# fanzyflani/pwnfps

Hardware: AMD Instinct MI355X
Metric: Mpixels/s at 3840x2160 (level.txt scene, trace + blur), frames resident on the device; mean steps/ray alongside; d2h_inclusive = the rate with every frame delivered to the host (SURVEY 8d) (higher is better)
Workload: dtype f32; 1 GPU; pwnfps level.txt scene (14 game.lua spheres, spawn pose, sec_current=0), 3840x2160, POSTPROC_BLUR=1, one frame per step; level=pwnfps_level, width=3840, height=2160, blur_passes=1, parallelism=rows/1, 3 frames in flight on two compute streams, frames_repeated_with_whole_strips=0

## Files before the change

### pwnfps_amd/csrc/pwn_api.cpp

```cpp
#include <hip/hip_runtime.h>
#include <stdint.h>
#include <stdio.h>
#include <stdlib.h>
#include <string.h>
#include <time.h>
#include <new>
#include <algorithm>
#include <vector>
#include <xmmintrin.h>

#include "pwnhip.h"
#include "pwn_internal.h"
#include "level_host.h"
#include "approx_tables.inc"

extern "C" const char *pwn_strerror(int code)
{
	switch(code)
	{
		case PWN_OK: return "ok";
		case PWN_EINVAL: return "invalid argument";
		case PWN_ENODEV: return "no usable HIP device";
		case PWN_ENOMEM: return "out of memory";
		case PWN_EIO: return "level file could not be read";
// ... 2 lines not shown
		case PWN_ETOOBIG: return "sphere tables exceed PWN_TABLES_MAX";
		case PWN_EBUSY: return "frame slot still in flight";
		case PWN_ENOTSUP: return "not available (RCCL missing, or not configured)";
		case PWN_ETIMEDOUT: return "the row tiling's deadline passed waiting for a peer";
	}
	return "unknown error";
}

extern "C" const char *pwn_last_error(pwn_ctx *ctx) { return ctx ? ctx->err : "null context"; }

static int ensure_scratch(pwn_ctx *c, size_t bytes)
{
	if(bytes <= c->scratch_cap) return PWN_OK;
	if(c->d_scratch) { (void)hipFree(c->d_scratch); c->d_scratch = NULL; c->scratch_cap = 0; }
	HIPCHK(c, hipMalloc((void **)&c->d_scratch, bytes));
	c->scratch_cap = bytes;
	return PWN_OK;
}

static void expand_tables(uint16_t *rcp, uint16_t *rsq);
static void frames_release(pwn_ctx *c);

#define GRP_HEAD(c) ((c) != NULL && (c)->grp != NULL && (c)->grp_head)
#define GRP_M0(c) pwn_group_member((c), 0)
#define GRP_REFUSE(c, what) do { if(GRP_HEAD(c)) { snprintf((c)->err, sizeof((c)->err), "%s is not available on a group's handle", what); return PWN_ENOTSUP; } } while(0)

extern "C" int pwn_init(pwn_ctx **out, int device, int width, int height)
{
	if(out == NULL || width <= 0 || height <= 0 || width > 32768 || height > 32768) return PWN_EINVAL;
	*out = NULL;
	int ndev = 0;
	if(hipGetDeviceCount(&ndev) != hipSuccess || ndev <= 0 || device < 0 || device >= ndev) return PWN_ENODEV;
	pwn_ctx *c = new(std::nothrow) pwn_ctx();
	if(c == NULL) return PWN_ENOMEM;
	c->device = device; c->w = width; c->h = height;
	c->blur_passes = 1; c->counters_on = 0; c->scheduler = PWN_SCHED_DEFAULT; c->refill_limit = PWN_REFILL_LIMIT_DEFAULT; c->have_level = false; c->cell_base_ok = false;
	if(const char *e = getenv("PWN_SCHEDULER")) c->scheduler = (strcmp(e, "refill") == 0 || strcmp(e, "1") == 0) ? PWN_SCHED_REFILL : PWN_SCHED_UNITS;
	if(const char *e = getenv("PWN_REFILL_LIMIT")) { int v = atoi(e); if(v >= 1 && v <= 64000) c->refill_limit = v; }
	c->dbg_force_hasw = getenv("PWN_DBG_FORCE_HASW") != NULL;
	c->dbg_blocks_per_cu = 0;
	c->dbg_blur_th = 0;
	if(const char *e = getenv("PWN_DBG_BLUR_TH")) c->dbg_blur_th = atoi(e);
	c->dbg_sphere_lists = 0; c->off_recsph = 0;
	c->dbg_sphere_lists = pwn_i_forced_lists();
	c->nbounds = 0;
	{ const char *e = getenv("PWN_SPHERE_BOUNDS"); c->dbg_sphere_bounds = (e != NULL && strcmp(e, "0") == 0) ? 0 : 1; }
	c->lists_form = PWN_LF_INDEXED; c->big_which = c->big_sph = 0; c->big_high = 0;
	for(int i = 0; i < PWN_NBLOB; i++) { c->d_big[i] = NULL; c->d_big_cap[i] = 0; }
	for(int i = 0; i < PWN_NSTAGE; i++) { c->h_big[i] = NULL; c->h_big_cap[i] = 0; }
	c->dbg_blur_tw = 0; c->dbg_blur_batch = -1;
	if(const char *e = getenv("PWN_DBG_BLUR_TW")) c->dbg_blur_tw = atoi(e);
	if(const char *e = getenv("PWN_DBG_BLUR_BATCH")) if(*e) c->dbg_blur_batch = atoi(e);
	if(const char *e = getenv("PWN_DBG_BLOCKS_PER_CU")) { int v = atoi(e); if(v > 0) c->dbg_blocks_per_cu = v; }
	c->blob_cur = 0; c->blob_dirty = true; c->off_sph = 0; c->stage_next = 0; c->up_stream = NULL;
	for(int i = 0; i < PWN_NBLOB; i++)
	{
		c->d_blob[i] = NULL; c->blob_has_static[i] = false;
		c->ev_tables[i] = NULL; c->tables_in_use[i] = false; c->tables_wait[i] = NULL;
		c->ev_upload[i] = NULL; c->upload_pending[i] = false;
	}
	for(int i = 0; i < PWN_NSTAGE; i++) { c->h_stage[i] = NULL; c->ev_stage[i] = NULL; c->stage_used[i] = false; }
	c->d_pre = c->d_out = NULL; c->d_z = NULL; c->d_skip = NULL; c->d_counters = NULL; c->d_tickets = NULL; c->ticket_set = 0; c->launch_rot = 2; c->launch_waits = 0;
	c->grid_reserve = 0;
	c->d_vpre = c->d_vout = NULL; c->d_vz = NULL; c->views_cap = 0; c->h_vrec = c->d_vrec = NULL; c->d_vrec_dev = NULL;
	c->d_ppre = c->d_pout = NULL; c->d_pz = NULL; c->h_prec = c->d_prec = NULL;
	c->h_rays = c->d_rays = NULL; c->rays_cap = 0;
	c->h_hits = c->d_hits = NULL; c->hits_cap = 0;
	memset(&c->room, 0, sizeof(c->room)); c->room.mode = -1;
	if(const char *e = getenv("PWN_TRACE_ROOM")) if(*e) c->room.mode = atoi(e) < 0 ? -1 : atoi(e);
	c->d_scratch = NULL; c->scratch_cap = 0;
	for(int i = 0; i < 12; i++) { c->occ_lds[i] = 0; c->occ_blocks[i] = 0; }
	c->stream = NULL; c->copy_stream = NULL; c->copy_stream2 = NULL; c->stream2 = NULL; c->d_pre2 = NULL;
	c->frame_overlap = 1; c->last_frame_done = NULL; c->last_frame_stream = NULL;
	if(const char *e = getenv("PWN_FRAME_OVERLAP")) c->frame_overlap = atoi(e) != 0;
	c->unit_order = 0;
	if(const char *e = getenv("PWN_UNIT_ORDER")) c->unit_order = atoi(e) != 0;
	c->tiled_comms = PWN_TILED_COMMS_ONE;
	if(const char *e = getenv("PWN_TILED_COMMS")) c->tiled_comms = (strcmp(e, "perstream") == 0 || strcmp(e, "2") == 0) ? PWN_TILED_COMMS_PER_STREAM : PWN_TILED_COMMS_ONE;
	c->tiled_streams = PWN_TILED_STREAMS_DEFAULT;
	if(const char *e = getenv("PWN_TILED_STREAMS")) { const int v = atoi(e); if(v == 2 || v == 3) c->tiled_streams = v; }
	c->tiled_choreo = PWN_TILED_CHOREO_INSTREAM;
	if(const char *e = getenv("PWN_TILED_CHOREO")) c->tiled_choreo = (strcmp(e, "split") == 0 || strcmp(e, "1") == 0) ? PWN_TILED_CHOREO_SPLIT : PWN_TILED_CHOREO_INSTREAM;
	memset(c->ev, 0, sizeof(c->ev));
	memset(&c->stats, 0, sizeof(c->stats));
	c->strip_reach = 0;
	c->call_strips = -1; c->strip_ev_n = 0; c->d_strip_miss = NULL; c->h_strip_miss = NULL; c->strip_backoff = 0;
	c->strip_calls = c->strip_redone = 0; c->strips_last = 1; c->host_regs_n = 0;
	memset(c->strip_ev, 0, sizeof(c->strip_ev));
	c->strip_copy_streams = 0; c->strip_calib_n = 0;
	if(const char *e = getenv("PWN_CALL_COPY_STREAMS")) if(atoi(e) == 1 || atoi(e) == 2) c->strip_copy_streams = atoi(e);
	if(const char *e = getenv("PWN_CALL_STRIPS")) if(*e) { const int v = atoi(e); if(v >= -1 && v <= PWN_CALL_STRIPS_MAX && v != 1) c->call_strips = v; }
	c->frame_timing = 1; c->wave_log_on = 0; c->d_wave_log = NULL; c->wave_log_cap = 0;
	c->nslots = 0; c->frame_flags = 0; c->frame_scale = 1; c->frame_pitch = 0; c->frame_seq = 0;
	memset(c->slot, 0, sizeof(c->slot));
	c->tiled = NULL; c->grp = NULL; c->grp_head = false; c->hub = NULL;
	c->err[0] = 0;
	pwn_level_clear(c->cells, c->pmap, c->spawn);
	c->bin_off.assign(4097, 0);
	expand_tables(c->tabs, c->tabs + 2048);

	int rc = PWN_OK;
	do
	{
		hipDeviceProp_t prop;
		if(hipSetDevice(device) != hipSuccess || hipGetDeviceProperties(&prop, device) != hipSuccess) { rc = PWN_ENODEV; break; }
		if(strncmp(prop.gcnArchName, "gfx950", 6) != 0)
// ... 838 lines not shown
		P.g_sph = (const float *)(c->d_big[cur] + c->big_sph);
	}
	P.nbounds = c->dbg_sphere_bounds ? c->nbounds : 0;
	for(int i = 0; i < PWN_BOUNDS_MAX; i++)
	{
		P.bound_ids[i] = 0xffffffffu;
		if(i < P.nbounds) { P.bounds[i] = c->bounds[i]; P.bound_ids[i] = c->bounds[i].id; }
	}
	if(c->upload_pending[cur])
	{
		if(hipEventQuery(c->ev_upload[cur]) == hipSuccess) c->upload_pending[cur] = false;
		else HIPCHK(c, hipStreamWaitEvent(stream, c->ev_upload[cur], 0));
	}
	P.counters = c->d_counters;
	P.clear_word = L->clear_word;
	P.cost_word = L->cost_word;
	P.wave_log = NULL;
	const unsigned rot = (unsigned)c->launch_rot, nsets = 2u * rot;
	P.tickets = c->d_tickets + (c->ticket_set % nsets) * PWN_QUEUES * PWN_QUEUE_STRIDE;
	P.tickets_next = c->d_tickets + ((c->ticket_set + rot) % nsets) * PWN_QUEUES * PWN_QUEUE_STRIDE;
	if(views != NULL) P.has_w = views->has_w;
	else if(rays != NULL) P.has_w = rays->has_w;
	else if(vps != NULL) P.has_w = vps->has_w;
	else P.has_w = camera_has_w(L->cam);
	if(c->dbg_force_hasw) P.has_w = 1;
	if(c->counters_on) HIPCHK(c, hipMemsetAsync(c->d_counters, 0, PWN_NCOUNTERS * sizeof(unsigned long long), stream));
	const bool refill = c->scheduler == PWN_SCHED_REFILL && !batch && !glb;
	const size_t lds_bytes = ((P.blob_bytes + 15u) & ~15u) + (refill ? pwn_trace_refill_lds_extra(P.has_w != 0) : pwn_trace_lds_extra());
	P.scheduler = c->scheduler;
	P.refill_limit = c->refill_limit;
	const int variant = (glb ? 8 : 0) | (refill ? 4 : 0) | (c->counters_on ? 2 : 0) | (P.has_w ? 1 : 0);
	if(c->occ_lds[variant] != lds_bytes)
	{
		c->occ_blocks[variant] = refill ? pwn_trace_refill_blocks_per_cu(lds_bytes, c->counters_on != 0, P.has_w != 0)
		                       : glb ? pwn_trace_global_blocks_per_cu(lds_bytes, c->counters_on != 0, P.has_w != 0)
		                             : pwn_trace_blocks_per_cu(lds_bytes, c->counters_on != 0, P.has_w != 0);
		c->occ_lds[variant] = lds_bytes;
	}
	int per_cu = c->occ_blocks[variant];
	{
		const int lds_fit = (int)(155648u / (((uint32_t)lds_bytes + 2047u) & ~2047u));
		if(per_cu > lds_fit) per_cu = lds_fit;
	}
	if(per_cu < 1) per_cu = 1;
	if(c->dbg_blocks_per_cu > 0) per_cu = c->dbg_blocks_per_cu;
	int grid = c->num_cus * per_cu;
	{
		const int room = c->room.mode >= 0 ? c->room.mode : L->room;
		const int reserve = c->grid_reserve > room ? c->grid_reserve : room;
		L->cost_mul = (uint32_t)grid;
		if(reserve > 0 && grid > 2 * reserve) grid -= reserve;
		L->cost_div = (uint32_t)grid;
	}
	{
		const int wg_waves = 4;
		if(!refill && grid > (P.tiles_total + wg_waves - 1) / wg_waves) grid = (P.tiles_total + wg_waves - 1) / wg_waves;
		if(grid > P.tiles_total) grid = P.tiles_total;
	}
	if(c->wave_log_on && !batch)
	{
		const size_t entries = (size_t)grid * 4 + 1;
		if(entries > c->wave_log_cap)
		{
			if(c->d_wave_log) { HIPCHK(c, hipDeviceSynchronize()); (void)hipFree(c->d_wave_log); c->d_wave_log = NULL; c->wave_log_cap = 0; }
			HIPCHK(c, hipMalloc((void **)&c->d_wave_log, entries * 16));
			c->wave_log_cap = entries;
		}
		HIPCHK(c, hipMemsetAsync(c->d_wave_log, 0, c->wave_log_cap * 16, stream));
		P.wave_log = c->d_wave_log;
	}
	const bool want_cost = !refill && !batch && !glb && (c->unit_order || (c->wave_log_on && getenv("PWN_DBG_UNIT_COST") != NULL));
	pwn_ctx::unit_order_state *uop = batch ? NULL : order_entry(c, stream, want_cost);
	if(uop != NULL && want_cost)
	{
		pwn_ctx::unit_order_state &uo = *uop;
		const size_t units = (size_t)P.tiles_total;
		const uint32_t qcap = (uint32_t)((units + PWN_QUEUES - 1u) / PWN_QUEUES);
		if(units > uo.cost_cap || (size_t)qcap * PWN_QUEUES > uo.perm_cap)
		{
			if(uo.d_cost || uo.d_perm) HIPCHK(c, hipDeviceSynchronize());
			(void)hipFree(uo.d_cost); (void)hipFree(uo.d_perm);
			uo.d_cost = NULL; uo.d_perm = NULL; uo.cost_cap = uo.perm_cap = 0; uo.perm_valid = uo.cost_fresh = false;
			HIPCHK(c, hipMalloc((void **)&uo.d_cost, units * 2));
			HIPCHK(c, hipMalloc((void **)&uo.d_perm, (size_t)qcap * PWN_QUEUES * 4));
			uo.cost_cap = units; uo.perm_cap = (size_t)qcap * PWN_QUEUES;
		}
		P.unit_cost = uo.d_cost;
		if(c->unit_order && uo.perm_valid && uo.perm_units == (uint32_t)units && uo.perm_y0 == y0 && uo.perm_y1 == y1)
		{
			P.perm = uo.d_perm; P.perm_cap = qcap;
			c->order_used++;
		}
		uo.units = (uint32_t)units; uo.qcap = qcap; uo.y0 = y0; uo.y1 = y1; uo.cost_fresh = true;
	}
	else if(uop != NULL) uop->cost_fresh = false;
	if(c->launch_event[rot - 1] != NULL && c->launch_stream[rot - 1] != stream)
	{
		HIPCHK(c, hipStreamWaitEvent(stream, c->launch_event[rot - 1], 0));
		c->launch_waits++;
	}
	if(refill) HIPCHK(c, pwn_launch_trace_refill(&P, grid, lds_bytes, c->counters_on != 0, stream));
	else HIPCHK(c, pwn_launch_trace(&P, grid, lds_bytes, c->counters_on != 0, stream));
	c->ticket_set++;
	c->launch_stream[2] = c->launch_stream[1]; c->launch_event[2] = c->launch_event[1];
	c->launch_stream[1] = c->launch_stream[0]; c->launch_event[1] = c->launch_event[0];
	c->launch_stream[0] = stream; c->launch_event[0] = caller_event != NULL ? caller_event : c->ev_tables[cur];
	if(caller_event != NULL)
	{
		for(int i = 0; i < PWN_NBLOB; i++)
			if(c->tables_in_use[i] && c->tables_wait[i] == caller_event) c->tables_in_use[i] = false;
		c->tables_wait[cur] = caller_event;
	}
	else
	{
		HIPCHK(c, hipEventRecord(c->ev_tables[cur], stream));
		c->tables_wait[cur] = c->ev_tables[cur];
	}
	c->tables_in_use[cur] = true;
	return PWN_OK;
}

int pwn_i_launch_order(pwn_ctx *c, hipStream_t stream)
{
	pwn_ctx::unit_order_state *uop = order_entry(c, stream, false);
// ... 1032 lines not shown
```

### pwnfps_amd/csrc/pwn_internal.h

```cpp
#pragma once
#include <hip/hip_runtime.h>
#include <stdint.h>
#include <stdio.h>
#include <vector>
#include <atomic>

#include "pwnhip.h"
#include "tables.h"

struct pwn_views_launch
{
	const pwn_view_rec *d_recs;
	int n;
	bool has_w;
	unsigned long long plane;
};

struct pwn_vps_launch
{
	const pwn_viewport_rec *d_recs, *h_recs;
	int n;
	bool has_w;
	uint32_t units;
};
// ... 124 lines not shown

	uint8_t cells[4096];
	uint32_t cell_base[65 * 65];
	bool cell_base_ok;
	uint32_t ep_recs[PWN_EP_MAX];
	pwn_portal pmap[26];
	int32_t spawn[2];
	std::vector<pwn_sphere> spheres;
	std::vector<int32_t> bin_off, bin_idx;
	std::vector<pwn_sphere> objs;
	std::vector<uint8_t> obj_typ;

	std::vector<uint8_t> blob;
	uint8_t *d_blob[PWN_NBLOB]; int blob_cur;
	bool blob_has_static[PWN_NBLOB];
	hipEvent_t ev_tables[PWN_NBLOB]; bool tables_in_use[PWN_NBLOB];
	hipEvent_t tables_wait[PWN_NBLOB];
	hipEvent_t ev_upload[PWN_NBLOB]; bool upload_pending[PWN_NBLOB];
	uint8_t *h_stage[PWN_NSTAGE]; hipEvent_t ev_stage[PWN_NSTAGE]; bool stage_used[PWN_NSTAGE]; unsigned stage_next;
	hipStream_t up_stream;
	uint16_t tabs[4096];
	uint32_t off_sph;
	uint32_t off_recsph; int dbg_sphere_lists;
	int lists_form;
	pwn_sphere_bound bounds[PWN_BOUNDS_MAX]; int nbounds;
	int dbg_sphere_bounds;
	std::vector<uint8_t> big; uint64_t big_which, big_sph;
	uint8_t *d_big[PWN_NBLOB]; size_t d_big_cap[PWN_NBLOB];
	uint8_t *h_big[PWN_NSTAGE]; size_t h_big_cap[PWN_NSTAGE];
	size_t big_high;
	bool blob_dirty;
	size_t occ_lds[12]; int occ_blocks[12];

	uint32_t *d_pre, *d_out;
	float *d_z;
	uint2 *d_skip;
	unsigned long long *d_counters;
	unsigned long long *d_wave_log; int wave_log_on; size_t wave_log_cap;
	struct unit_order_state
	{
		hipStream_t key; bool used; unsigned long long stamp;
		uint16_t *d_cost; uint32_t *d_perm; size_t cost_cap, perm_cap;
		uint32_t units, qcap; int y0, y1;
		bool cost_fresh;
		uint32_t perm_units; int perm_y0, perm_y1; bool perm_valid;
	} order[4];
	unsigned long long order_stamp;
	int tiled_choreo;
	int tiled_streams;
	int tiled_comms;
	int unit_order;
	unsigned long long order_used, order_sorts;
	bool dbg_force_hasw; int dbg_blocks_per_cu;
	int dbg_blur_th, dbg_blur_tw, dbg_blur_batch;
	int grid_reserve;
	uint32_t *d_vpre, *d_vout; float *d_vz; int views_cap;
	pwn_view_rec *h_vrec, *d_vrec;
	pwn_view_rec *d_vrec_dev;
	uint32_t *d_ppre, *d_pout; float *d_pz;
	pwn_viewport_rec *h_prec, *d_prec;
	unsigned char *h_rays, *d_rays; size_t rays_cap;
	unsigned char *h_hits, *d_hits; size_t hits_cap;
	uint32_t *d_tickets; unsigned ticket_set;
	uint32_t *d_scratch; size_t scratch_cap;

	hipStream_t stream;
	hipStream_t stream2;
	uint32_t *d_pre2;
	pwn_room_ctl room;
	int frame_overlap;
	hipEvent_t last_frame_done; hipStream_t last_frame_stream;
	hipStream_t copy_stream;
	hipEvent_t ev[4];
	int call_strips;
	hipStream_t copy_stream2;
	int strip_copy_streams;
	int strip_calib_n; double strip_calib_ms[16];
	hipEvent_t strip_ev[2 * PWN_CALL_STRIPS_MAX]; int strip_ev_n;
	uint32_t *d_strip_miss, *h_strip_miss;
	int strips_last;
	int strip_reach;
	int strip_backoff;
	unsigned long long strip_calls, strip_redone;
	struct host_reg { void *base; size_t bytes; } host_regs[PWN_HOST_REGS_MAX]; int host_regs_n;
	pwn_stats stats;

	int nslots, frame_flags, frame_scale, frame_pitch, frame_timing;
	pwn_slot slot[PWN_MAX_SLOTS];
	uint64_t frame_seq;

	pwn_group *grp; bool grp_head;
	pwn_hub *hub;
	pwn_tiled *tiled;
	int tiled_init_ms, tiled_wait_ms;

	hipStream_t launch_stream[3]; hipEvent_t launch_event[3];
	unsigned long long launch_waits;
	int launch_rot;

	char err[256];
};

#define HIPCHK(ctx, call) do { hipError_t e_ = (call); if(e_ != hipSuccess) { \
	snprintf((ctx)->err, sizeof((ctx)->err), "%s: %s", #call, hipGetErrorString(e_)); return PWN_EHIP; } } while(0)

int pwn_i_launch_trace(pwn_ctx *c, pwn_trace_launch *L);
// ... 44 lines not shown
```

### pwnfps_amd/csrc/tables.h

```cpp
#pragma once
#include <stdint.h>
#include "cell_bake.h"
#include "sphere_bound.h"

#define PWN_GRID_PITCH 65u
#define PWN_T_RCP      0u
#define PWN_T_RSQ      4096u
#define PWN_T_FACES    8192u
#define PWN_T_EXP2     8448u
#define PWN_T_CELLINFO 8704u
#define PWN_T_EPREC    25616u
#define PWN_T_BINIDX   25824u

#define PWN_RCP_BASE   0x7e800000u
#define PWN_RSQ_BASE   0x5f000000u

#define PWN_C_ROOM   0x0100u
#define PWN_C_ROOM2  0x0200u
#define PWN_C_FOG    0x0400u
#define PWN_C_DQ     0x0800u
#define PWN_C_RAMP   0x1000u
#define PWN_C_RAMPX  0x2000u
#define PWN_C_RAMPM  0x4000u
#define PWN_C_PORTAL 0x8000u
// ... 57 lines not shown
		case '$': return PWN_C_ROOM | PWN_C_FOG;
		case '"': return PWN_C_ROOM | PWN_C_DQ;
		case '#': return PWN_C_ROOM | PWN_C_ROOM2;
		case '&': return PWN_C_ROOM | PWN_C_ROOM2 | PWN_C_FOG;
		case '>': return PWN_C_RAMP | PWN_C_RAMPX | PWN_C_RAMPM;
		case '<': return PWN_C_RAMP | PWN_C_RAMPX;
		case ',': return PWN_C_RAMP | PWN_C_RAMPM;
		case '^': return PWN_C_RAMP;
	}
	return (c >= 'A' && c <= 'Z') ? PWN_C_PORTAL : 0u;
}

struct pwn_trace_params
{
	float rayb[4], rdx[4], rdy[4], from[4];
	float sec_current;
	int w, h, y0, y1;
	int tiles_x, tiles_total;
	uint32_t ux_magic; int ux_shift;
	uint32_t blob_bytes, off_sph;
	uint32_t *sbuf;
	float *zbuf;
	const uint32_t *blob;
	unsigned long long *counters;
	unsigned long long *wave_log;
	int has_w;
	int scheduler;
	int refill_limit;
	uint32_t *tickets, *tickets_next;
	uint32_t *cost_word;
	uint16_t *unit_cost;
	const uint32_t *perm;
	uint32_t perm_cap;
	uint32_t *clear_word;
	uint32_t off_recsph;
	const struct pwn_view_rec *views;
	int nviews;
	uint32_t views_magic; int views_shift;
	unsigned long long plane;
	const float *rays;
	const uint32_t *ray_seeds;
	uint32_t nrays;
	int ray_w;
	void *hits;
	const float *g_rec;
	const uint32_t *g_which;
	const float *g_sph;
	const struct pwn_viewport_rec *vps;
	int nvp;
	uint32_t vp_step0;
	int nbounds;
	uint32_t bound_ids[PWN_BOUNDS_MAX];
	pwn_sphere_bound bounds[PWN_BOUNDS_MAX];
};
#define PWN_HIT_REC_BYTES 48u

struct pwn_blur_params
{
	int w, h, y0, y1;
	int groups;
	const uint32_t *pre;
	const float *zbuf;
	uint32_t *out;
	const uint2 *skip;
	int avail_y0, avail_y1;
	uint32_t *miss;
	int tile_h, tile_w, batch;
	uint32_t *cost_acc, *cost_out;
	uint32_t cost_mul, cost_div;
	int views;
	unsigned long long plane;
	const struct pwn_viewport_rec *vps;
	int nvp, vp_tiles;
};

enum { PWN_KM_FRAME = 0, PWN_KM_VIEWS = 1, PWN_KM_RAYS = 2, PWN_KM_HITS = 3, PWN_KM_VIEWPORTS = 4 };

struct pwn_view_rec
{
	float rayb[4], rdx[4], rdy[4], from[4];
	float sec_current;
	float pad_[3];
};
#define PWN_VIEWS_REC_BYTES 80u

struct pwn_viewport_rec
{
	float rayb[4], rdx[4], rdy[4], from[4];
	float sec_current;
	int32_t x, y, w, h;
	uint32_t units_x; uint32_t ux_magic; int32_t ux_shift;
	uint32_t rows_u;
	uint32_t units;
	uint32_t seg_first, seg_round, seg_magic; int32_t seg_shift;
	uint32_t pad_[2];
};
#define PWN_VP_REC_BYTES 128u

#ifndef PWN_QUEUES
#define PWN_QUEUES 64u
#endif
#define PWN_QUEUE_STRIDE 32u
```

### pwnfps_amd/csrc/trace_common.h

```cpp
#pragma once
#include <hip/hip_runtime.h>
#include <mutex>
#include "dev_math.h"
#include "tables.h"

#define EPS 0.0000000000001f
#define REFLECT_BLUR_F 0.03f
#define REFLECT_MAX 2
enum { FXP = 0, FZP, FXN, FZN, FYP, FYN };

#ifndef PWN_BLOCK
#define PWN_BLOCK 256
#endif
#define TILE_W 16
#define TILE_H 4

#ifndef PWN_MIN_WAVES
#define PWN_MIN_WAVES 3
#endif

#define PWN_LDS __attribute__((address_space(3)))
#define PWN_KARGS __attribute__((address_space(4)))
template<class T> __device__ __forceinline__ const PWN_LDS T *lds_at(uint32_t byte) { return (const PWN_LDS T *)(uintptr_t)byte; }
typedef float pwn_f4 __attribute__((ext_vector_type(4)));
// ... 62 lines not shown

static_assert(PWN_C_PST_SHIFT == 2u && PWN_T_EPREC + PWN_EP_MAX * 4u <= PWN_T_BINIDX, "ep_rec takes the state field as a byte offset; 52 records fit");
static_assert(PWN_C_RAMPX == (1u << PWN_C_PROT_SHIFT) && PWN_C_RAMPM == (2u << PWN_C_PROT_SHIFT), "the rotation takes the place of RAMPX | RAMPM");
static_assert(pwn_cell_class('A') == PWN_C_PORTAL && pwn_cell_class('M') == PWN_C_PORTAL && pwn_cell_class('Z') == PWN_C_PORTAL, "a letter's cell has no ramp bit");
static_assert((PWN_C_PST_MASK | PWN_C_LT2 | PWN_C_LTDQ) == 0xffu, "the baked byte lies below the class bits");
typedef _Float16 pwn_h2 __attribute__((ext_vector_type(2)));
__device__ __forceinline__ pwn_h2 ep_rec(const Lds &L, uint32_t pst_in_place)
{
	return __builtin_bit_cast(pwn_h2, *(const PWN_LDS uint32_t *)(L.eprec + pst_in_place));
}

template<bool HAS_W> struct Vec { float x, y, z, w; };

template<bool W> __device__ __forceinline__ float dot3(const Vec<W> &a, const Vec<W> &b)
{
	if constexpr(W) return (a.x * b.x + a.z * b.z) + (a.y * b.y + a.w * b.w);
	else return (a.x * b.x + a.z * b.z) + a.y * b.y;
}
template<bool W> __device__ __forceinline__ Vec<W> vscale(float s, const Vec<W> &a)
{
	Vec<W> r; r.x = s * a.x; r.y = s * a.y; r.z = s * a.z;
	if constexpr(W) r.w = s * a.w; else r.w = 0.0f;
	return r;
}
template<bool W> __device__ __forceinline__ Vec<W> vadd(const Vec<W> &a, const Vec<W> &b)
{
	Vec<W> r; r.x = a.x + b.x; r.y = a.y + b.y; r.z = a.z + b.z;
	if constexpr(W) r.w = a.w + b.w; else r.w = 0.0f;
	return r;
}
template<bool W> __device__ __forceinline__ Vec<W> vsub(const Vec<W> &a, const Vec<W> &b)
{
	Vec<W> r; r.x = a.x - b.x; r.y = a.y - b.y; r.z = a.z - b.z;
	if constexpr(W) r.w = a.w - b.w; else r.w = 0.0f;
	return r;
}
template<bool W> __device__ __forceinline__ Vec<W> vnormalise(const PWN_LDS uint16_t *rsq, const Vec<W> &a)
{
	return vscale<W>(tab_rsqrt(rsq, dot3<W>(a, a)), a);
}

__device__ __forceinline__ float dpp_row_shr1(float v)
{
	return __int_as_float(__builtin_amdgcn_update_dpp(0, __float_as_int(v), 0x111 , 0xf, 0xf, true));
}

enum { EV_NONE = 0, EV_WALL, EV_SPHERE, EV_EXHAUSTED };
enum { BASE_CEIL = 0, BASE_FLOOR, BASE_WALL, BASE_MAGENTA, BASE_ROOM_Y };

enum { RG_SEG = 0, RG_SETUP_SLOW, RG_EXHAUSTED, RG_WALL, RG_SPHERE, RG_FLOOR, RG_SPHREFL, RG_JITTER, RG_COMP1, RG_COMP1_FOG,
	RG_COMP2, RG_COMP2_FOG, RG_HELP, RG_UNIT, RG_SPHTEST, RG_SPHUPD, RG_ELSE,
	RG_UNIT_HALF, RG_HC_R2, RG_HC_OUT, RG_PORTAL_WALL, RG_PORTAL_GO, RG_PORTAL_ODD, RG_PORTAL_ROT2,
	RG_SPHBOUND, RG_SPHSKIP,
	RG_N };
struct Counters { uint32_t rays, steps, portals, tests, exhausted, wsteps, wp[8], apasses, apass_lanes, rg[RG_N]; };
#define WAVE_PATH(k) do { if(COUNT && (__ffsll((long long)__ballot(1)) - 1) == (int)(threadIdx.x & 63)) cnt.wp[k]++; } while(0)
#define RG(k) do { if(COUNT && (__ffsll((long long)__ballot(1)) - 1) == (int)(threadIdx.x & 63)) cnt.rg[k]++; } while(0)


__device__ __forceinline__ uint32_t pixel_seed(int x, int y, int w)
{
	uint32_t seed = (uint32_t)x + (uint32_t)y * (uint32_t)y * ((uint32_t)w + 1u);
	seed *= seed * seed;
	seed *= seed * seed;
	return seed << 1;
}

__device__ __forceinline__ void blob_to_lds(unsigned char *lds, const void *blob, uint32_t blob_bytes)
{
	const uint4 *src = (const uint4 *)blob;
	uint4 *dst = (uint4 *)lds;
	int n16 = (int)(blob_bytes >> 4);
	for(int i = threadIdx.x; i < n16; i += PWN_BLOCK) dst[i] = src[i];
}

__device__ __forceinline__ uint32_t next_open_queue(uint32_t q, unsigned long long open)
{
	static_assert(PWN_QUEUES <= 64u && (PWN_QUEUES & (PWN_QUEUES - 1u)) == 0u, "a power of two, one lane per queue");
	if constexpr(PWN_QUEUES == 64u)
	{
		const uint32_t rot = q + 1u;
		const unsigned long long r = rot == 64u ? open : ((open >> rot) | (open << (64u - rot)));
		return (q + 1u + (uint32_t)__builtin_ctzll(r)) & 63u;
	}
	else
		return (q + 1u + (uint32_t)__builtin_ctzll((open | (open << (PWN_QUEUES & 31u))) >> (q + 1u))) & (PWN_QUEUES - 1u);
}

__device__ __forceinline__ unsigned long long *wave_log_slot(unsigned long long *wave_log)
{
	static_assert(PWN_BLOCK == 256, "one wave per SIMD: simd_id tells the waves of a workgroup apart");
	const unsigned simd = __builtin_amdgcn_s_getreg(4 | (4 << 6) | ((2 - 1) << 11));
	const size_t wid = 1u + (size_t)blockIdx.x * 4u + simd;
	return wave_log + 2 * wid;
}
__device__ __forceinline__ bool wave_first_lane()
{
	return __builtin_amdgcn_mbcnt_hi(~0u, __builtin_amdgcn_mbcnt_lo(~0u, 0u)) == 0u;
}


template<auto KERNEL>
static hipError_t launch_kernel(const pwn_trace_params *P, int grid, size_t lds_bytes, hipStream_t stream)
{
	static size_t lds_mark[64];
	static std::mutex lds_lock;
// ... 46 lines not shown
```

### pwnfps_amd/csrc/trace_kernel.hip

```cpp
#include <hip/hip_runtime.h>
#include "trace_common.h"

#define WALK_STEPS 1000
#define EV_OUT_OF_STEPS 0
#define WALK_EV_KEEP ev
#define WALK_EV_OPEN(e) ((e) <= 0)

template<bool COUNT, bool HAS_W, int LISTS>
__device__ __forceinline__ void trace_pixel(const Lds &L, float sec_current, uint32_t seed,
	Vec<HAS_W> from, Vec<HAS_W> iray, float &out_x, float &out_y, float &out_z, float &out_w,
	float *zpix, Counters &cnt)
{
	typedef Vec<HAS_W> V;
	constexpr bool HITREC = false;
	[[maybe_unused]] uint32_t hit_cxz;
	[[maybe_unused]] int hit_portals;
	float st_refl0, st_refl1, st_fog0, st_fog1;
	float sc0x = 1.0f, sc0y = 1.0f, sc0z = 1.0f;
	float sc1x, sc1y, sc1z;
	asm volatile("" : "=v"(st_refl0)); asm volatile("" : "=v"(st_refl1)); asm volatile("" : "=v"(st_fog0)); asm volatile("" : "=v"(st_fog1));
	asm volatile("" : "=v"(sc1x)); asm volatile("" : "=v"(sc1y)); asm volatile("" : "=v"(sc1z));
#define icx sc0x
#define icy sc0y
#define icz sc0z
// ... 126 lines not shown
			at = aux_pos;
		}
		r0 = make_uint4((uint32_t)ev, (uint32_t)ldir, (uint32_t)object, (uint32_t)hit_portals);
		r1 = make_uint4(__float_as_uint(dist), __float_as_uint(at.x), __float_as_uint(at.y), __float_as_uint(at.z));
		r2 = make_uint4(__float_as_uint(ray.x), __float_as_uint(ray.y), __float_as_uint(ray.z), hit_cxz);
	}
	out[0] = r0; out[1] = r1; out[2] = r2;
}

#define PWN_CHAIN_ROUND3(m) "s_mov_b32 exec_lo, " m "\n\ts_mov_b32 exec_hi, " m "\n\tv_add_f32 %0, %4, %0\n\tv_add_f32 %1, %5, %1\n\tv_add_f32 %2, %6, %2\n\t"
#define PWN_CHAIN_ROUND4(m) "s_mov_b32 exec_lo, " m "\n\ts_mov_b32 exec_hi, " m "\n\tv_add_f32 %0, %5, %0\n\tv_add_f32 %1, %6, %1\n\tv_add_f32 %2, %7, %2\n\tv_add_f32 %3, %8, %3\n\t"
#define PWN_CHAIN_ALL(R) R("0xfffefffe") R("0xfffcfffc") R("0xfff8fff8") R("0xfff0fff0") R("0xffe0ffe0") R("0xffc0ffc0") R("0xff80ff80") \
	R("0xff00ff00") R("0xfe00fe00") R("0xfc00fc00") R("0xf800f800") R("0xf000f000") R("0xe000e000") R("0xc000c000") R("0x80008000")
template<bool HAS_W> __device__ __forceinline__ void chain_rounds(Vec<HAS_W> &v, const Vec<HAS_W> &rdx)
{
	unsigned long long saved;
	if constexpr(HAS_W)
		asm volatile("s_mov_b64 %4, exec\n\t" PWN_CHAIN_ALL(PWN_CHAIN_ROUND4) "s_mov_b64 exec, %4"
			: "+v"(v.x), "+v"(v.y), "+v"(v.z), "+v"(v.w), "=&s"(saved) : "s"(rdx.x), "s"(rdx.y), "s"(rdx.z), "s"(rdx.w));
	else
		asm volatile("s_mov_b64 %3, exec\n\t" PWN_CHAIN_ALL(PWN_CHAIN_ROUND3) "s_mov_b64 exec, %3"
			: "+v"(v.x), "+v"(v.y), "+v"(v.z), "=&s"(saved) : "s"(rdx.x), "s"(rdx.y), "s"(rdx.z));
}

template<bool COUNT, bool HAS_W, bool ORDER, int LISTS, int MODE>
__global__ void __launch_bounds__(PWN_BLOCK, PWN_MIN_WAVES)
pwn_trace_kernel(pwn_trace_params P)
{
	constexpr bool VIEWS = MODE == PWN_KM_VIEWS, HITS = MODE == PWN_KM_HITS, RAYS = MODE == PWN_KM_RAYS || HITS, VPS = MODE == PWN_KM_VIEWPORTS;
	extern __shared__ __attribute__((aligned(16))) unsigned char lds_raw[];

	blob_to_lds(lds_raw, P.blob, P.blob_bytes);
	if(threadIdx.x == 0) *(uint32_t *)(lds_raw + ((P.blob_bytes + 15u) & ~15u)) = 0u;
	__syncthreads();

	const Lds L = LISTS == PWN_LF_GLOBAL ? lds_tables_global(P) : lds_tables(P.off_sph, P.off_recsph);

	typedef Vec<HAS_W> V;
	V rayb, rdx, rdy, from;
	rayb.x = P.rayb[0]; rayb.y = P.rayb[1]; rayb.z = P.rayb[2]; rayb.w = HAS_W ? P.rayb[3] : 0.0f;
	rdx.x = P.rdx[0]; rdx.y = P.rdx[1]; rdx.z = P.rdx[2]; rdx.w = HAS_W ? P.rdx[3] : 0.0f;
	rdy.x = P.rdy[0]; rdy.y = P.rdy[1]; rdy.z = P.rdy[2]; rdy.w = HAS_W ? P.rdy[3] : 0.0f;
	from.x = P.from[0]; from.y = P.from[1]; from.z = P.from[2]; from.w = HAS_W ? P.from[3] : 1.0f;
	float sec_current = P.sec_current;

	const int lane = threadIdx.x & 63, wave = threadIdx.x >> 6;
	const int l16 = lane & 15;

	Counters cnt = {};
	unsigned long long t_begin = 0ull;
	if(P.wave_log != NULL || P.cost_word != NULL) t_begin = __builtin_amdgcn_s_memrealtime();

	const uint32_t units_x = ((uint32_t)P.w + 15u) >> 4;
	const uint32_t units = VPS ? (uint32_t)P.tiles_total : RAYS ? (P.nrays + 63u) >> 6 : units_x * (((uint32_t)(P.y1 - P.y0) + 3u) >> 2) * (VIEWS ? (uint32_t)P.nviews : 1u);
	if(blockIdx.x == 0 && threadIdx.x < PWN_QUEUES) P.tickets_next[threadIdx.x * PWN_QUEUE_STRIDE] = 0u;
	if(blockIdx.x == 0 && threadIdx.x == PWN_QUEUES && P.clear_word != NULL) *P.clear_word = 0u;
	uint32_t q = (blockIdx.x * (PWN_BLOCK / 64) + (uint32_t)wave) % PWN_QUEUES;
	uint32_t ticket;
	const uint32_t nwaves_all = gridDim.x * (PWN_BLOCK / 64);
#define QBASE(qq) ((nwaves_all + PWN_QUEUES - 1u - (qq)) / PWN_QUEUES)
	ticket = (blockIdx.x * (PWN_BLOCK / 64) + (uint32_t)wave) / PWN_QUEUES;
	int misses = 0;
#ifdef PWN_DRAW_PROBE
	unsigned long long probe_ticks = 0ull, probe_n = 0ull;
#endif
	const uint32_t draw_n = units >= 16u * (PWN_BLOCK / 64u) * gridDim.x ? 2u : 1u;
	uint32_t left = 0u;
	for(;;)
	{
		const uint32_t qlen = (units + PWN_QUEUES - 1u - q) / PWN_QUEUES;
		if(ticket >= qlen)
		{
			RG(RG_HELP);
			if(++misses > 2 * (int)PWN_QUEUES) break;
			left = 0u;
			uint32_t seen = 0xffffffffu;
			uint32_t ql = 0u;
			asm volatile("" : "+v"(ql));
			ql = __builtin_amdgcn_mbcnt_hi(~0u, __builtin_amdgcn_mbcnt_lo(~0u, ql));
			if(ql < PWN_QUEUES)
				seen = __hip_atomic_load(&P.tickets[ql * PWN_QUEUE_STRIDE], __ATOMIC_RELAXED, __HIP_MEMORY_SCOPE_AGENT);
			const uint32_t len_l = (units + PWN_QUEUES - 1u - (ql & (PWN_QUEUES - 1u))) / PWN_QUEUES;
			const unsigned long long open = __ballot(ql < PWN_QUEUES && seen < len_l - min(len_l, QBASE(ql & (PWN_QUEUES - 1u))));
			if(open == 0ull) break;
			q = next_open_queue(q, open);
			uint32_t t = 0;
			if(lane == 0) t = atomicAdd(&P.tickets[q * PWN_QUEUE_STRIDE], 1u);
			ticket = (uint32_t)__builtin_amdgcn_readfirstlane((int)t) + QBASE(q);
			continue;
		}
		RG(RG_UNIT);
		misses = 0;
		uint32_t ln;
		if constexpr(HAS_W)
		{
			ln = 0u;
			asm volatile("" : "+v"(ln));
			ln = __builtin_amdgcn_mbcnt_hi(~0u, __builtin_amdgcn_mbcnt_lo(~0u, ln));
		}
		else ln = (uint32_t)lane;
		uint32_t unit = ticket * PWN_QUEUES + q;
		if(ORDER && P.perm != NULL)
		{
			const uint32_t *pp = P.perm + (uint32_t)__builtin_amdgcn_readfirstlane((int)(q * P.perm_cap + ticket));
			asm volatile("s_load_dword %0, %1, 0x0\n\ts_waitcnt lgkmcnt(0)" : "=s"(unit) : "s"(pp) : "memory");
		}
		const bool draw = left == 0u;
		uint32_t next_raw = ticket + 1u;
#ifndef PWN_DRAW_PROBE
		if(draw && ln == 0u) next_raw = atomicAdd(&P.tickets[q * PWN_QUEUE_STRIDE], draw_n) + QBASE(q);
#else
		if(RAYS && draw && ln == 0u) next_raw = atomicAdd(&P.tickets[q * PWN_QUEUE_STRIDE], draw_n) + QBASE(q);
#endif
		if constexpr(RAYS)
		{
			const uint32_t i = unit * 64u + ln;
			if(i < P.nrays)
			{
				const pwn_f4 *rec = (const pwn_f4 *)P.rays + 2u * (size_t)i;
				const pwn_f4 o = rec[0], d = rec[1];
				uint32_t seed = 0u;
				if constexpr(!HITS)
				{
					seed = P.ray_seeds != NULL ? P.ray_seeds[i] : 0u;
					seed <<= 1;
				}
				V org, dir;
				org.x = o.x; org.y = o.y; org.z = o.z; org.w = HAS_W && P.ray_w ? o.w : 1.0f;
				dir.x = d.x; dir.y = d.y; dir.z = d.z; dir.w = HAS_W && P.ray_w ? d.w : 0.0f;
				if constexpr(HITS)
				{
					trace_hit<COUNT, HAS_W, LISTS>(L, org, dir, (uint4 *)((unsigned char *)P.hits + (size_t)i * PWN_HIT_REC_BYTES), cnt);
				}
				else
				{
					float ox, oy, oz, ow;
					trace_pixel<COUNT, HAS_W, LISTS>(L, sec_current, seed, org, dir, ox, oy, oz, ow, P.zbuf + i, cnt);
					P.sbuf[i] = col_pack4(ox, oy, oz, ow);
				}
			}
			ticket = (uint32_t)__builtin_amdgcn_readfirstlane((int)next_raw);
			left = draw ? draw_n - 1u : left - 1u;
			continue;
		}
		uint32_t fu = unit;
		uint32_t *sbuf = P.sbuf;
		float *zbuf = P.zbuf;
		if constexpr(VIEWS)
		{
			fu = P.views_shift >= 0 ? __umulhi(unit, P.views_magic) >> P.views_shift : unit;
			const uint32_t view = (uint32_t)__builtin_amdgcn_readfirstlane((int)(unit - fu * (uint32_t)P.nviews));
			typedef const __attribute__((address_space(4))) float cfloat;
			const cfloat *r = (const cfloat *)((uintptr_t)P.views + (uintptr_t)view * PWN_VIEWS_REC_BYTES);
			rayb.x = r[0]; rayb.y = r[1]; rayb.z = r[2]; rayb.w = HAS_W ? r[3] : 0.0f;
			rdx.x = r[4]; rdx.y = r[5]; rdx.z = r[6]; rdx.w = HAS_W ? r[7] : 0.0f;
			rdy.x = r[8]; rdy.y = r[9]; rdy.z = r[10]; rdy.w = HAS_W ? r[11] : 0.0f;
			from.x = r[12]; from.y = r[13]; from.z = r[14]; from.w = HAS_W ? r[15] : 1.0f;
			sec_current = r[16];
			sbuf += (size_t)view * (size_t)P.plane;
			zbuf += (size_t)view * (size_t)P.plane;
		}
		int fw = P.w, fh = P.h, fy0 = P.y0, fy1 = P.y1;
		uint32_t fux = units_x, fmagic = P.ux_magic;
		int fshift = P.ux_shift;
		uint32_t rows_u = ((uint32_t)(P.y1 - P.y0) + 3u) >> 2;
		uint32_t org = 0u;
		if constexpr(VPS)
		{
			typedef const __attribute__((address_space(4))) uint32_t cu32;
			typedef const __attribute__((address_space(4))) float cfloat;
			const uintptr_t base = (uintptr_t)P.vps;
			const uint32_t t = (uint32_t)__builtin_amdgcn_readfirstlane((int)unit), nvp = (uint32_t)P.nvp;
			uint32_t s = 0u;
			for(uint32_t step = P.vp_step0; step != 0u; step >>= 1)
			{
				const uint32_t c = min(s + step, nvp - 1u);
				const uint32_t first = ((cu32 *)(base + (uintptr_t)c * PWN_VP_REC_BYTES))[26];
				if(s + step < nvp && first <= t) s += step;
			}
			cu32 *sr = (cu32 *)(base + (uintptr_t)s * PWN_VP_REC_BYTES);
			const uint32_t d = t - sr[26], cnt = nvp - s;
			const int sshift = (int)sr[29];
			const uint32_t rr = sshift >= 0 ? __umulhi(d, sr[28]) >> sshift : d;
			const uint32_t view = s + (d - rr * cnt);
			fu = sr[27] + rr;
			cu32 *ri = (cu32 *)(base + (uintptr_t)view * PWN_VP_REC_BYTES);
			const cfloat *r = (const cfloat *)ri;
			rayb.x = r[0]; rayb.y = r[1]; rayb.z = r[2]; rayb.w = HAS_W ? r[3] : 0.0f;
			rdx.x = r[4]; rdx.y = r[5]; rdx.z = r[6]; rdx.w = HAS_W ? r[7] : 0.0f;
			rdy.x = r[8]; rdy.y = r[9]; rdy.z = r[10]; rdy.w = HAS_W ? r[11] : 0.0f;
			from.x = r[12]; from.y = r[13]; from.z = r[14]; from.w = HAS_W ? r[15] : 1.0f;
			sec_current = r[16];
			fw = (int)ri[19]; fh = (int)ri[20]; fy0 = 0; fy1 = fh;
			fux = ri[21]; fmagic = ri[22]; fshift = (int)ri[23]; rows_u = ri[24];
			org = ri[18] * (uint32_t)P.w + ri[17];
		}
		uint32_t k;
		if(fshift >= 0) k = __umulhi(fu, fmagic) >> fshift;
		else k = fu;
		const uint32_t ux = fu - k * fux;
		const int hrow = ((fh >> 1) - fy0) >> 2;
		const uint32_t mid = (uint32_t)min(max(hrow, 0), (int)rows_u - 1);
		uint32_t uy;
		{
			const uint32_t a = mid, b = rows_u - 1u - mid, m = min(a, b);
			const uint32_t j = (k + 1u) >> 1;
			if(k <= 2u * m) uy = (k & 1u) ? mid - j : mid + j;
			else uy = a > b ? mid - (k - b) : mid + (k - a);
		}
		const int half = (int)(ux & 1u);
		const int cx0 = (int)(ux >> 1) * 32;
		const int x = (int)ux * 16 + (HAS_W ? (int)(ln & 15u) : l16), y = fy0 + (int)uy * 4 + (HAS_W ? (int)(ln >> 4) : (lane >> 4));

		V rayl = vadd<HAS_W>(vadd<HAS_W>(vscale<HAS_W>((float)cx0, rdx), rayb), vscale<HAS_W>((float)y, rdy));
		if(half)
		{
			RG(RG_UNIT_HALF);
#pragma unroll
			for(int k = 0; k < 16; k++) rayl = vadd<HAS_W>(rayl, rdx);
		}
		rayl = vadd<HAS_W>(rayl, rdx);
#ifndef PWN_CHAIN_DPP
		chain_rounds<HAS_W>(rayl, rdx);
#else
		{
			const bool first = (l16 == 0);
			V add;
			add.x = first ? rayl.x : rdx.x; add.y = first ? rayl.y : rdx.y; add.z = first ? rayl.z : rdx.z;
			add.w = HAS_W ? (first ? rayl.w : rdx.w) : 0.0f;
#pragma unroll
			for(int k = 1; k < 16; k++)
			{
				rayl.x = dpp_row_shr1(rayl.x) + add.x;
				rayl.y = dpp_row_shr1(rayl.y) + add.y;
				rayl.z = dpp_row_shr1(rayl.z) + add.z;
				if constexpr(HAS_W) rayl.w = dpp_row_shr1(rayl.w) + add.w;
			}
		}
#endif

		unsigned long long u_begin = 0ull;
		if(ORDER && P.unit_cost != NULL) u_begin = __builtin_amdgcn_s_memrealtime();
		if(x < fw && y < fy1)
		{
			const uint32_t seed = pixel_seed(x, y, fw);
			float ox, oy, oz, ow;
			const uint32_t o = __umul24((uint32_t)y, (uint32_t)P.w) + (uint32_t)x + org;
			trace_pixel<COUNT, HAS_W, LISTS>(L, sec_current, seed, from, rayl, ox, oy, oz, ow, zbuf + o, cnt);
			sbuf[o] = col_pack4(ox, oy, oz, ow);
		}
		if(ORDER && P.unit_cost != NULL && ln == 0u)
		{
			const unsigned long long d = (__builtin_amdgcn_s_memrealtime() - u_begin) >> 2;
			P.unit_cost[unit] = (uint16_t)(d > 65535ull ? 65535ull : d);
		}
#ifdef PWN_DRAW_PROBE
		{
			const unsigned long long p0 = __builtin_amdgcn_s_memrealtime();
			if(draw && lane == 0) next_raw = atomicAdd(&P.tickets[q * PWN_QUEUE_STRIDE], draw_n) + QBASE(q);
			ticket = (uint32_t)__builtin_amdgcn_readfirstlane((int)next_raw);
			asm volatile("" : "+s"(ticket));
			probe_ticks += __builtin_amdgcn_s_memrealtime() - p0;
			probe_n++;
		}
#else
		ticket = (uint32_t)__builtin_amdgcn_readfirstlane((int)next_raw);
#endif
		left = draw ? draw_n - 1u : left - 1u;
	}

	if(COUNT)
	{
#define PWN_CNT_REGIONS RG_N
#include "trace_counters.inc"
#undef PWN_CNT_REGIONS
		if(lane == 0) atomicAdd(&P.counters[16 + RG_N], 1ull);
	}
	if(P.wave_log != NULL && wave_first_lane())
	{
		unsigned long long *wl = wave_log_slot(P.wave_log);
#ifdef PWN_DRAW_PROBE
		wl[0] = probe_ticks | (probe_n << 40); wl[1] = __builtin_amdgcn_s_memrealtime() - t_begin;
#else
		wl[0] = t_begin; wl[1] = __builtin_amdgcn_s_memrealtime();
#endif
	}
	if(P.cost_word != NULL && wave_first_lane())
	{
		static_assert(PWN_BLOCK == 256, "four waves per workgroup");
		const uint32_t life = (uint32_t)(__builtin_amdgcn_s_memrealtime() - t_begin) & 0x03ffffffu;
		PWN_LDS uint32_t *wg = (PWN_LDS uint32_t *)(uintptr_t)((P.blob_bytes + 15u) & ~15u);
		const uint32_t old = __hip_atomic_fetch_add(wg, life + (1u << 28), __ATOMIC_RELAXED, __HIP_MEMORY_SCOPE_WORKGROUP);
		if((old >> 28) == 3u) (void)__hip_atomic_fetch_add(P.cost_word, (old + life) & 0x0fffffffu, __ATOMIC_RELAXED, __HIP_MEMORY_SCOPE_AGENT);
	}
}

template<bool ORDER, int LISTS, int MODE>
using Units = TraceKernels<pwn_trace_kernel<true, true, ORDER, LISTS, MODE>, pwn_trace_kernel<true, false, ORDER, LISTS, MODE>,
	pwn_trace_kernel<false, true, ORDER, LISTS, MODE>, pwn_trace_kernel<false, false, ORDER, LISTS, MODE>>;

extern "C" hipError_t pwn_launch_trace(const pwn_trace_params *P, int grid, size_t lds_bytes, bool count, hipStream_t stream)
{
// ... 35 lines not shown
```

Baseline: 28510 Mpixels/s.

## Pair adjacent horizontal tiles per wave work item, carrying ray state across

Each ticketed work unit now covers two horizontally adjacent 16x4 tiles in the lower rows of the frame, except for a band of single-tile rows kept for load balance. The second tile's ray directions are continued from the first tile's end values via ds_bpermute instead of being rebuilt, and the ticket draw count drops to one when pairing. The aim is to halve the ticket atomics and the per-unit setup cost, at the price of coarser scheduling granularity and possible tail imbalance. Floating-point accumulation of the ray direction now runs through 32 pixels instead of 16, which can slightly change the rays produced.

```diff
diff --git a/pwnfps_amd/csrc/pwn_api.cpp b/pwnfps_amd/csrc/pwn_api.cpp
--- a/pwnfps_amd/csrc/pwn_api.cpp
+++ b/pwnfps_amd/csrc/pwn_api.cpp
@@ -78,6 +78,8 @@
 	if(const char *e = getenv("PWN_DBG_BLUR_TW")) c->dbg_blur_tw = atoi(e);
 	if(const char *e = getenv("PWN_DBG_BLUR_BATCH")) if(*e) c->dbg_blur_batch = atoi(e);
 	if(const char *e = getenv("PWN_DBG_BLOCKS_PER_CU")) { int v = atoi(e); if(v > 0) c->dbg_blocks_per_cu = v; }
+	c->tile_pairs = 1;
+	if(const char *e = getenv("PWN_TILE_PAIRS")) if(*e) { const int v = atoi(e); if(v >= 0 && v <= 2) c->tile_pairs = v; }
 	c->blob_cur = 0; c->blob_dirty = true; c->off_sph = 0; c->stage_next = 0; c->up_stream = NULL;
 	for(int i = 0; i < PWN_NBLOB; i++)
 	{
@@ -1022,10 +1024,28 @@
 		if(reserve > 0 && grid > 2 * reserve) grid -= reserve;
 		L->cost_div = (uint32_t)grid;
 	}
+	const bool want_cost = !refill && !batch && !glb && (c->unit_order || (c->wave_log_on && getenv("PWN_DBG_UNIT_COST") != NULL));
+	int items = P.tiles_total;
+	if(!refill && !batch && !want_cost && (c->tile_pairs == 2 || (c->tile_pairs == 1 && (long long)P.tiles_total >= 16ll * 4 * grid)))
+	{
+		const int tx = (P.tiles_x + 1) / 2;
+		P.tile_pairs = 1;
+		unit_div_magic((uint32_t)tx, &P.tx_magic, &P.tx_shift);
+		const int rows = P.tiles_total / P.tiles_x;
+		int single = 0;
+		if(c->tile_pairs != 2)
+		{
+			single = (4 * grid + P.tiles_x - 1) / P.tiles_x;
+			if(single < (rows + 4) / 5) single = (rows + 4) / 5;
+		}
+		if(single > rows) single = rows;
+		P.pair_single_rows = single;
+		items = single * P.tiles_x + tx * (rows - single);
+	}
 	{
 		const int wg_waves = 4;
-		if(!refill && grid > (P.tiles_total + wg_waves - 1) / wg_waves) grid = (P.tiles_total + wg_waves - 1) / wg_waves;
-		if(grid > P.tiles_total) grid = P.tiles_total;
+		if(!refill && grid > (items + wg_waves - 1) / wg_waves) grid = (items + wg_waves - 1) / wg_waves;
+		if(grid > items) grid = items;
 	}
 	if(c->wave_log_on && !batch)
 	{
@@ -1039,7 +1059,6 @@
 		HIPCHK(c, hipMemsetAsync(c->d_wave_log, 0, c->wave_log_cap * 16, stream));
 		P.wave_log = c->d_wave_log;
 	}
-	const bool want_cost = !refill && !batch && !glb && (c->unit_order || (c->wave_log_on && getenv("PWN_DBG_UNIT_COST") != NULL));
 	pwn_ctx::unit_order_state *uop = batch ? NULL : order_entry(c, stream, want_cost);
 	if(uop != NULL && want_cost)
 	{
diff --git a/pwnfps_amd/csrc/pwn_internal.h b/pwnfps_amd/csrc/pwn_internal.h
--- a/pwnfps_amd/csrc/pwn_internal.h
+++ b/pwnfps_amd/csrc/pwn_internal.h
@@ -200,6 +200,7 @@
 	int unit_order;
 	unsigned long long order_used, order_sorts;
 	bool dbg_force_hasw; int dbg_blocks_per_cu;
+	int tile_pairs;
 	int dbg_blur_th, dbg_blur_tw, dbg_blur_batch;
 	int grid_reserve;
 	uint32_t *d_vpre, *d_vout; float *d_vz; int views_cap;
diff --git a/pwnfps_amd/csrc/tables.h b/pwnfps_amd/csrc/tables.h
--- a/pwnfps_amd/csrc/tables.h
+++ b/pwnfps_amd/csrc/tables.h
@@ -133,6 +133,9 @@
 	int nbounds;
 	uint32_t bound_ids[PWN_BOUNDS_MAX];
 	pwn_sphere_bound bounds[PWN_BOUNDS_MAX];
+	int tile_pairs;
+	uint32_t tx_magic; int tx_shift;
+	int pair_single_rows;
 };
 #define PWN_HIT_REC_BYTES 48u
 
diff --git a/pwnfps_amd/csrc/trace_common.h b/pwnfps_amd/csrc/trace_common.h
--- a/pwnfps_amd/csrc/trace_common.h
+++ b/pwnfps_amd/csrc/trace_common.h
@@ -138,6 +138,7 @@
 	RG_COMP2, RG_COMP2_FOG, RG_HELP, RG_UNIT, RG_SPHTEST, RG_SPHUPD, RG_ELSE,
 	RG_UNIT_HALF, RG_HC_R2, RG_HC_OUT, RG_PORTAL_WALL, RG_PORTAL_GO, RG_PORTAL_ODD, RG_PORTAL_ROT2,
 	RG_SPHBOUND, RG_SPHSKIP,
+	RG_UNIT_RIGHT,
 	RG_N };
 struct Counters { uint32_t rays, steps, portals, tests, exhausted, wsteps, wp[8], apasses, apass_lanes, rg[RG_N]; };
 #define WAVE_PATH(k) do { if(COUNT && (__ffsll((long long)__ballot(1)) - 1) == (int)(threadIdx.x & 63)) cnt.wp[k]++; } while(0)
diff --git a/pwnfps_amd/csrc/trace_kernel.hip b/pwnfps_amd/csrc/trace_kernel.hip
--- a/pwnfps_amd/csrc/trace_kernel.hip
+++ b/pwnfps_amd/csrc/trace_kernel.hip
@@ -202,7 +202,15 @@
 	if(P.wave_log != NULL || P.cost_word != NULL) t_begin = __builtin_amdgcn_s_memrealtime();
 
 	const uint32_t units_x = ((uint32_t)P.w + 15u) >> 4;
-	const uint32_t units = VPS ? (uint32_t)P.tiles_total : RAYS ? (P.nrays + 63u) >> 6 : units_x * (((uint32_t)(P.y1 - P.y0) + 3u) >> 2) * (VIEWS ? (uint32_t)P.nviews : 1u);
+	constexpr bool PAIRABLE = MODE == PWN_KM_FRAME && !ORDER;
+	const bool pairs = PAIRABLE && P.tile_pairs != 0;
+	const uint32_t tiles_x = (units_x + 1u) >> 1;
+	uint32_t pair_shift = (uint32_t)__builtin_amdgcn_readfirstlane(pairs ? 1 : 0);
+	asm volatile("" : "+s"(pair_shift));
+	const uint32_t rows_all = ((uint32_t)(P.y1 - P.y0) + 3u) >> 2;
+	const uint32_t single_rows = (uint32_t)__builtin_amdgcn_readfirstlane((int)(pairs ? min((uint32_t)P.pair_single_rows, rows_all) : rows_all));
+	const uint32_t pair_first = (uint32_t)__builtin_amdgcn_readfirstlane((int)(single_rows * units_x));
+	const uint32_t units = VPS ? (uint32_t)P.tiles_total : RAYS ? (P.nrays + 63u) >> 6 : (pair_first + tiles_x * (rows_all - single_rows)) * (VIEWS ? (uint32_t)P.nviews : 1u);
 	if(blockIdx.x == 0 && threadIdx.x < PWN_QUEUES) P.tickets_next[threadIdx.x * PWN_QUEUE_STRIDE] = 0u;
 	if(blockIdx.x == 0 && threadIdx.x == PWN_QUEUES && P.clear_word != NULL) *P.clear_word = 0u;
 	uint32_t q = (blockIdx.x * (PWN_BLOCK / 64) + (uint32_t)wave) % PWN_QUEUES;
@@ -214,7 +222,7 @@
 #ifdef PWN_DRAW_PROBE
 	unsigned long long probe_ticks = 0ull, probe_n = 0ull;
 #endif
-	const uint32_t draw_n = units >= 16u * (PWN_BLOCK / 64u) * gridDim.x ? 2u : 1u;
+	const uint32_t draw_n = !pairs && units >= 16u * (PWN_BLOCK / 64u) * gridDim.x ? 2u : 1u;
 	uint32_t left = 0u;
 	for(;;)
 	{
@@ -239,7 +247,6 @@
 			ticket = (uint32_t)__builtin_amdgcn_readfirstlane((int)t) + QBASE(q);
 			continue;
 		}
-		RG(RG_UNIT);
 		misses = 0;
 		uint32_t ln;
 		if constexpr(HAS_W)
@@ -313,6 +320,8 @@
 		int fw = P.w, fh = P.h, fy0 = P.y0, fy1 = P.y1;
 		uint32_t fux = units_x, fmagic = P.ux_magic;
 		int fshift = P.ux_shift;
+		uint32_t kbase = 0u, ush = 0u;
+		if(PAIRABLE && pair_shift != 0u && (uint32_t)__builtin_amdgcn_readfirstlane((int)unit) >= pair_first) { fu -= pair_first; fux = tiles_x; fmagic = P.tx_magic; fshift = P.tx_shift; kbase = single_rows; ush = 1u; }
 		uint32_t rows_u = ((uint32_t)(P.y1 - P.y0) + 3u) >> 2;
 		uint32_t org = 0u;
 		if constexpr(VPS)
@@ -348,7 +357,8 @@
 		uint32_t k;
 		if(fshift >= 0) k = __umulhi(fu, fmagic) >> fshift;
 		else k = fu;
-		const uint32_t ux = fu - k * fux;
+		const uint32_t ux = (fu - k * fux) << (PAIRABLE ? ush : 0u);
+		if(PAIRABLE) k += kbase;
 		const int hrow = ((fh >> 1) - fy0) >> 2;
 		const uint32_t mid = (uint32_t)min(max(hrow, 0), (int)rows_u - 1);
 		uint32_t uy;
@@ -360,44 +370,78 @@
 		}
 		const int half = (int)(ux & 1u);
 		const int cx0 = (int)(ux >> 1) * 32;
-		const int x = (int)ux * 16 + (HAS_W ? (int)(ln & 15u) : l16), y = fy0 + (int)uy * 4 + (HAS_W ? (int)(ln >> 4) : (lane >> 4));
-
-		V rayl = vadd<HAS_W>(vadd<HAS_W>(vscale<HAS_W>((float)cx0, rdx), rayb), vscale<HAS_W>((float)y, rdy));
+
+		V rayl = vadd<HAS_W>(vadd<HAS_W>(vscale<HAS_W>((float)cx0, rdx), rayb), vscale<HAS_W>((float)(fy0 + (int)uy * 4 + (HAS_W ? (int)(ln >> 4) : (lane >> 4))), rdy));
 		if(half)
 		{
 			RG(RG_UNIT_HALF);
 #pragma unroll
 			for(int k = 0; k < 16; k++) rayl = vadd<HAS_W>(rayl, rdx);
 		}
-		rayl = vadd<HAS_W>(rayl, rdx);
-#ifndef PWN_CHAIN_DPP
-		chain_rounds<HAS_W>(rayl, rdx);
-#else
-		{
-			const bool first = (l16 == 0);
-			V add;
-			add.x = first ? rayl.x : rdx.x; add.y = first ? rayl.y : rdx.y; add.z = first ? rayl.z : rdx.z;
-			add.w = HAS_W ? (first ? rayl.w : rdx.w) : 0.0f;
-#pragma unroll
-			for(int k = 1; k < 16; k++)
+		float carry = 0.0f;
+		int x = (int)ux * 16 + (HAS_W ? (int)(ln & 15u) : l16), y = fy0 + (int)uy * 4 + (HAS_W ? (int)(ln >> 4) : (lane >> 4));
+		bool right_next = PAIRABLE && ush != 0u && (uint32_t)__builtin_amdgcn_readfirstlane((int)ux) + 1u < units_x;
+		unsigned long long u_begin = 0ull;
+#pragma unroll 1
+		for(;;)
+		{
+			RG(RG_UNIT);
+			rayl = vadd<HAS_W>(rayl, rdx);
+			chain_rounds<HAS_W>(rayl, rdx);
+			if(PAIRABLE && right_next)
 			{
-				rayl.x = dpp_row_shr1(rayl.x) + add.x;
-				rayl.y = dpp_row_shr1(rayl.y) + add.y;
-				rayl.z = dpp_row_shr1(rayl.z) + add.z;
-				if constexpr(HAS_W) rayl.w = dpp_row_shr1(rayl.w) + add.w;
+				uint32_t lp;
+				if constexpr(HAS_W)
+				{
+					lp = 0u;
+					asm volatile("" : "+v"(lp));
+					lp = __builtin_amdgcn_mbcnt_hi(~0u, __builtin_amdgcn_mbcnt_lo(~0u, lp));
+				}
+				else lp = (uint32_t)lane;
+				const int src = (int)(((lp & 3u) << 6) | 60u);
+				const int px = __builtin_amdgcn_ds_bpermute(src, __float_as_int(rayl.x));
+				const int py = __builtin_amdgcn_ds_bpermute(src, __float_as_int(rayl.y));
+				const int pz = __builtin_amdgcn_ds_bpermute(src, __float_as_int(rayl.z));
+				int pc = lp < 4u ? px : lp < 8u ? py : pz;
+				if constexpr(HAS_W)
+				{
+					const int pw = __builtin_amdgcn_ds_bpermute(src, __float_as_int(rayl.w));
+					pc = lp < 12u ? pc : pw;
+				}
+				const int xy = (x - (int)(lp & 15u)) | ((y - (int)(lp >> 4)) << 16);
+				carry = __int_as_float(lp < 16u ? pc : xy);
 			}
-		}
-#endif
-
-		unsigned long long u_begin = 0ull;
-		if(ORDER && P.unit_cost != NULL) u_begin = __builtin_amdgcn_s_memrealtime();
-		if(x < fw && y < fy1)
-		{
-			const uint32_t seed = pixel_seed(x, y, fw);
-			float ox, oy, oz, ow;
-			const uint32_t o = __umul24((uint32_t)y, (uint32_t)P.w) + (uint32_t)x + org;
-			trace_pixel<COUNT, HAS_W, LISTS>(L, sec_current, seed, from, rayl, ox, oy, oz, ow, zbuf + o, cnt);
-			sbuf[o] = col_pack4(ox, oy, oz, ow);
+			if(ORDER && P.unit_cost != NULL) u_begin = __builtin_amdgcn_s_memrealtime();
+			if(x < fw && y < fy1)
+			{
+				const uint32_t seed = pixel_seed(x, y, fw);
+				float ox, oy, oz, ow;
+				const uint32_t o = __umul24((uint32_t)y, (uint32_t)P.w) + (uint32_t)x + org;
+				trace_pixel<COUNT, HAS_W, LISTS>(L, sec_current, seed, from, rayl, ox, oy, oz, ow, zbuf + o, cnt);
+				sbuf[o] = col_pack4(ox, oy, oz, ow);
+			}
+			if(!(PAIRABLE && right_next)) break;
+			RG(RG_UNIT_RIGHT);
+			right_next = false;
+			{
+				uint32_t lp;
+				if constexpr(HAS_W)
+				{
+					lp = 0u;
+					asm volatile("" : "+v"(lp));
+					lp = __builtin_amdgcn_mbcnt_hi(~0u, __builtin_amdgcn_mbcnt_lo(~0u, lp));
+				}
+				else lp = (uint32_t)lane;
+				const int ci = __float_as_int(carry);
+				const int dst = (int)((lp >> 4) << 2);
+				rayl.x = __int_as_float(__builtin_amdgcn_ds_bpermute(dst, ci));
+				rayl.y = __int_as_float(__builtin_amdgcn_ds_bpermute(dst + 16, ci));
+				rayl.z = __int_as_float(__builtin_amdgcn_ds_bpermute(dst + 32, ci));
+				if constexpr(HAS_W) rayl.w = __int_as_float(__builtin_amdgcn_ds_bpermute(dst + 48, ci));
+				const int xy = __builtin_amdgcn_readlane(ci, 16);
+				x = (xy & 0xffff) + 16 + (int)(lp & 15u);
+				y = (xy >> 16) + (int)(lp >> 4);
+			}
 		}
 		if(ORDER && P.unit_cost != NULL && ln == 0u)
 		{
```

New measurement: 30420 Mpixels/s, median of 6. +6.7%, better.
